# NVlabs/EmerNeRF

Measured on NVIDIA H100. Metric: training rays/sec (8192-ray batch), higher is better.
Workload: dtype f32

## Files before the change

emernerf_b200/csrc/field_fused.cu:

```cuda
#include "common.cuh"
#include "tc_common.cuh"

namespace emer {
namespace ff {

using namespace emer::tc;

constexpr int ROWS = 64;
constexpr int WGS = 3;
constexpr int THREADS = WGS * 128;
constexpr int H = 64;

struct FwdParams {
    const float* enc; int64_t ld_enc; int k_enc;
    const float *wb0, *bb0, *wb1, *bb1; int n_feat;
    const float* w0g; int64_t ld_w0;
    const float *w1h, *w1g; int64_t ld_w1;
    const float *w2, *b2;
    const float* ray_bias; int samples;
    float *sigma, *rgb;
    float *save_hb, *save_hg, *save_h1, *save_sem;
    int64_t n;
};

struct Smem {
    int wb0_hi, wb0_lo, wb1_hi, wb1_lo, wg_hi, wg_lo, w1h_hi, w1h_lo, w2_hi, w2_lo, bias, total;
};
__host__ __device__ inline Smem smem_map(int k_enc, int n_feat) {
    Smem m;
    int o = 0;
    const int wb0 = (k_enc / 4) * H * 16, wb1 = (H / 4) * n_feat * 16, wg = (H / 4) * 128 * 16, w1h = (H / 4) * H * 16,
              w2 = (H / 4) * 8 * 16;
    m.wb0_hi = o; o += wb0; m.wb0_lo = o; o += wb0;
    m.wb1_hi = o; o += wb1; m.wb1_lo = o; o += wb1;
    m.wg_hi = o; o += wg; m.wg_lo = o; o += wg;
    m.w1h_hi = o; o += w1h; m.w1h_lo = o; o += w1h;
    m.w2_hi = o; o += w2; m.w2_lo = o; o += w2;
    m.bias = o; o += (64 + 128 + 4) * 4;
    m.total = o;
    return m;
}

__device__ __forceinline__ void stage_weight(uint8_t* hi, uint8_t* lo, const float* __restrict__ w, int64_t ld, int rows,
                                             int rows_valid, int k_valid, int row0, int tid) {
    for (int e = tid; e < rows_valid * k_valid; e += THREADS) {
        const int r = e / k_valid, k = e - r * k_valid;
        float h, l;
        split(__ldg(w + (int64_t)r * ld + k), h, l);
        const int off = b_off(row0 + r, k, rows);
        *reinterpret_cast<float*>(hi + off) = h;
        *reinterpret_cast<float*>(lo + off) = l;
    }
}
__device__ __forceinline__ void stage_weight_t(uint8_t* hi, uint8_t* lo, const float* __restrict__ w, int64_t ld, int rows,
                                               int rows_valid, int k_valid, int row0, int tid) {
    for (int e = tid; e < rows_valid * k_valid; e += THREADS) {
        const int o = e / rows_valid, j = e - o * rows_valid;
        float h, l;
        split(__ldg(w + (int64_t)o * ld + j), h, l);
        const int off = b_off(row0 + j, o, rows);
        *reinterpret_cast<float*>(hi + off) = h;
        *reinterpret_cast<float*>(lo + off) = l;
    }
}

__device__ __forceinline__ float2 ld2(const float* p, bool ok) {
    return ok ? __ldg(reinterpret_cast<const float2*>(p)) : make_float2(0.f, 0.f);
}
__device__ __forceinline__ void st2(float* p, float a, float b, bool ok) {
    if (ok) *reinterpret_cast<float2*>(p) = make_float2(a, b);
}

__device__ __forceinline__ void relu_back(float (&acc)[32], const float* saved, float* dst, int64_t ld, int64_t row0,
                                          int64_t row1, bool ok0, bool ok1, int q, uint32_t (&ahi)[8][4],
                                          uint32_t (&alo)[8][4]) {
#pragma unroll
    for (int j = 0; j < 8; ++j) {
        const int c = 8 * j + 2 * q;
        const float2 m0 = ld2(saved + row0 * ld + c, ok0), m1 = ld2(saved + row1 * ld + c, ok1);
        acc[4 * j] = m0.x > 0.f ? acc[4 * j] : 0.f;
        acc[4 * j + 1] = m0.y > 0.f ? acc[4 * j + 1] : 0.f;
        acc[4 * j + 2] = m1.x > 0.f ? acc[4 * j + 2] : 0.f;
        acc[4 * j + 3] = m1.y > 0.f ? acc[4 * j + 3] : 0.f;
        st2(dst + row0 * ld + c, acc[4 * j], acc[4 * j + 1], ok0);
        st2(dst + row1 * ld + c, acc[4 * j + 2], acc[4 * j + 3], ok1);
        frag_split(acc[4 * j], acc[4 * j + 1], acc[4 * j + 2], acc[4 * j + 3], ahi[j], alo[j]);
    }
}

__device__ __forceinline__ void ray_colsum(const float (&v)[32], float* dst, int lane, bool live) {
#pragma unroll
    for (int j = 0; j < 8; ++j) {
#pragma unroll
        for (int e = 0; e < 2; ++e) {
            float s = v[4 * j + e] + v[4 * j + 2 + e];
            s += __shfl_xor_sync(0xffffffffu, s, 4);
            s += __shfl_xor_sync(0xffffffffu, s, 8);
            s += __shfl_xor_sync(0xffffffffu, s, 16);
            if (lane < 4 && live) atomicAdd(dst + 8 * j + 2 * lane + e, s);
        }
    }
}

template <int K_ENC, int NF>
__global__ void __launch_bounds__(THREADS, 1) field_fwd_kernel(const FwdParams p) {
    extern __shared__ __align__(128) uint8_t smem[];
    const Smem m = smem_map(K_ENC, NF);
    float* bias_s = reinterpret_cast<float*>(smem + m.bias);
    const int tid = threadIdx.x;

    for (int i = tid * 16; i < m.bias; i += THREADS * 16) *reinterpret_cast<float4*>(smem + i) = make_float4(0.f, 0.f, 0.f, 0.f);
    __syncthreads();
    stage_weight(smem + m.wb0_hi, smem + m.wb0_lo, p.wb0, K_ENC, H, H, K_ENC, 0, tid);
    stage_weight(smem + m.wb1_hi, smem + m.wb1_lo, p.wb1, H, NF, NF, H, 0, tid);
    stage_weight(smem + m.wg_hi, smem + m.wg_lo, p.w0g, p.ld_w0, 128, H, H, 0, tid);
    stage_weight(smem + m.wg_hi, smem + m.wg_lo, p.w1g, p.ld_w1, 128, H, H, H, tid);
    stage_weight(smem + m.w1h_hi, smem + m.w1h_lo, p.w1h, p.ld_w1, H, H, H, 0, tid);
    stage_weight(smem + m.w2_hi, smem + m.w2_lo, p.w2, H, 8, 3, H, 0, tid);
    for (int e = tid; e < 64 + 128 + 4; e += THREADS) {
        float v = 0.0f;
        if (e < 64) v = __ldg(p.bb0 + e);
        else if (e < 64 + 128) { if (e - 64 < NF) v = __ldg(p.bb1 + e - 64); }
        else if (e - 192 < 3) v = __ldg(p.b2 + e - 192);
        bias_s[e] = v;
    }
    fence_async_proxy();
    __syncthreads();

    const uint32_t sb = smem_u32(smem);
    const int wg = tid >> 7, w = (tid >> 5) & 3, lane = tid & 31, q = lane & 3;
    const float* bb0_s = bias_s;
    const float* bb1_s = bias_s + 64;
    const float* b2_s = bias_s + 192;
    const int64_t n_tiles = (p.n + ROWS - 1) / ROWS;

    for (int64_t tile = (int64_t)blockIdx.x * WGS + wg; tile < n_tiles; tile += (int64_t)gridDim.x * WGS) {
        const int64_t row0 = tile * ROWS + 16 * w + (lane >> 2), row1 = row0 + 8;
        const bool ok0 = row0 < p.n, ok1 = row1 < p.n;
        uint32_t ahi[8][4], alo[8][4];

#pragma unroll
        for (int j = 0; j < K_ENC / 8; ++j) {
            const float2 x0 = ld2(p.enc + row0 * p.ld_enc + 8 * j + 2 * q, ok0);
            const float2 x1 = ld2(p.enc + row1 * p.ld_enc + 8 * j + 2 * q, ok1);
            frag_split(x0.x, x0.y, x1.x, x1.y, ahi[j], alo[j]);
        }
        float acc[32];
        wg_fence();
#pragma unroll
        for (int ks = 0; ks < K_ENC / 8; ++ks)
            mma3<64>(acc, ahi[ks], alo[ks], b_desc(sb + m.wb0_hi, H, ks, 0), b_desc(sb + m.wb0_lo, H, ks, 0), ks > 0);
        wg_commit();
        wg_wait0();
#pragma unroll
        for (int j = 0; j < 8; ++j) {
            const int c = 8 * j + 2 * q;
            const float v0 = fmaxf(acc[4 * j] + bb0_s[c], 0.0f), v1 = fmaxf(acc[4 * j + 1] + bb0_s[c + 1], 0.0f);
            const float v2 = fmaxf(acc[4 * j + 2] + bb0_s[c], 0.0f), v3 = fmaxf(acc[4 * j + 3] + bb0_s[c + 1], 0.0f);
            if (p.save_hb) {
                st2(p.save_hb + row0 * H + c, v0, v1, ok0);
                st2(p.save_hb + row1 * H + c, v2, v3, ok1);
            }
            frag_split(v0, v1, v2, v3, ahi[j], alo[j]);
        }

        float geo[32], sem[NF > H ? 32 : 1];
        wg_fence();
#pragma unroll
        for (int ks = 0; ks < 8; ++ks) {
            mma3<64>(geo, ahi[ks], alo[ks], b_desc(sb + m.wb1_hi, NF, ks, 0), b_desc(sb + m.wb1_lo, NF, ks, 0), ks > 0);
            if constexpr (NF > H)
                mma3<64>(sem, ahi[ks], alo[ks], b_desc(sb + m.wb1_hi, NF, ks, H), b_desc(sb + m.wb1_lo, NF, ks, H), ks > 0);
        }
        wg_commit();
        wg_wait0();
#pragma unroll
        for (int j = 0; j < 8; ++j) {
            const int c = 8 * j + 2 * q;
            const float v0 = geo[4 * j] + bb1_s[c], v1 = geo[4 * j + 1] + bb1_s[c + 1];
            const float v2 = geo[4 * j + 2] + bb1_s[c], v3 = geo[4 * j + 3] + bb1_s[c + 1];
            if (j == 0 && q == 0) {
                if (ok0) p.sigma[row0] = expf(v0 - 1.0f);
                if (ok1) p.sigma[row1] = expf(v2 - 1.0f);
            }
            if (p.save_hg) {
                st2(p.save_hg + row0 * 128 + H + c, v0, v1, ok0);
                st2(p.save_hg + row1 * 128 + H + c, v2, v3, ok1);
            }
            frag_split(v0, v1, v2, v3, ahi[j], alo[j]);
        }
        if constexpr (NF > H) {
#pragma unroll
            for (int j = 0; j < 8; ++j) {
                const int c = 8 * j + 2 * q;
                st2(p.save_sem + row0 * H + c, sem[4 * j] + bb1_s[H + c], sem[4 * j + 1] + bb1_s[H + c + 1], ok0);
                st2(p.save_sem + row1 * H + c, sem[4 * j + 2] + bb1_s[H + c], sem[4 * j + 3] + bb1_s[H + c + 1], ok1);
            }
        }

        float d0[32], d1[32];
        wg_fence();
#pragma unroll
        for (int ks = 0; ks < 8; ++ks) {
            mma3<64>(d0, ahi[ks], alo[ks], b_desc(sb + m.wg_hi, 128, ks, 0), b_desc(sb + m.wg_lo, 128, ks, 0), ks > 0);
            mma3<64>(d1, ahi[ks], alo[ks], b_desc(sb + m.wg_hi, 128, ks, H), b_desc(sb + m.wg_lo, 128, ks, H), ks > 0);
        }
        wg_commit();
        wg_wait0();
        const float* rb0 = p.ray_bias + ((ok0 ? row0 : p.n - 1) / p.samples) * 128;
        const float* rb1 = p.ray_bias + ((ok1 ? row1 : p.n - 1) / p.samples) * 128;
#pragma unroll
        for (int j = 0; j < 8; ++j) {
            const int c = 8 * j + 2 * q;
            const float2 b0 = __ldg(reinterpret_cast<const float2*>(rb0 + c)), b1 = __ldg(reinterpret_cast<const float2*>(rb1 + c));
            const float v0 = fmaxf(d0[4 * j] + b0.x, 0.0f), v1 = fmaxf(d0[4 * j + 1] + b0.y, 0.0f);
            const float v2 = fmaxf(d0[4 * j + 2] + b1.x, 0.0f), v3 = fmaxf(d0[4 * j + 3] + b1.y, 0.0f);
            if (p.save_hg) {
                st2(p.save_hg + row0 * 128 + c, v0, v1, ok0);
                st2(p.save_hg + row1 * 128 + c, v2, v3, ok1);
            }
            frag_split(v0, v1, v2, v3, ahi[j], alo[j]);
        }

        wg_fence();
#pragma unroll
        for (int ks = 0; ks < 8; ++ks)
            mma3<64>(d1, ahi[ks], alo[ks], b_desc(sb + m.w1h_hi, H, ks, 0), b_desc(sb + m.w1h_lo, H, ks, 0), 1);
        wg_commit();
        wg_wait0();
#pragma unroll
        for (int j = 0; j < 8; ++j) {
            const int c = 8 * j + 2 * q;
            const float2 b0 = __ldg(reinterpret_cast<const float2*>(rb0 + H + c));
            const float2 b1 = __ldg(reinterpret_cast<const float2*>(rb1 + H + c));
            const float v0 = fmaxf(d1[4 * j] + b0.x, 0.0f), v1 = fmaxf(d1[4 * j + 1] + b0.y, 0.0f);
            const float v2 = fmaxf(d1[4 * j + 2] + b1.x, 0.0f), v3 = fmaxf(d1[4 * j + 3] + b1.y, 0.0f);
            if (p.save_h1) {
                st2(p.save_h1 + row0 * H + c, v0, v1, ok0);
                st2(p.save_h1 + row1 * H + c, v2, v3, ok1);
            }
            frag_split(v0, v1, v2, v3, ahi[j], alo[j]);
        }

        float d2[4];
        wg_fence();
#pragma unroll
        for (int ks = 0; ks < 8; ++ks)
            mma3<8>(d2, ahi[ks], alo[ks], b_desc(sb + m.w2_hi, 8, ks, 0), b_desc(sb + m.w2_lo, 8, ks, 0), ks > 0);
        wg_commit();
        wg_wait0();
#pragma unroll
        for (int e = 0; e < 2; ++e) {
            const int c = 2 * q + e;
            if (c < 3) {
                if (ok0) p.rgb[row0 * 3 + c] = 1.0f / (1.0f + expf(-(d2[e] + b2_s[c])));
                if (ok1) p.rgb[row1 * 3 + c] = 1.0f / (1.0f + expf(-(d2[2 + e] + b2_s[c])));
            }
        }
    }
}


struct BwdParams {
    const float *d_rgb, *rgb, *d_sigma, *sigma, *d_geo, *d_sem;
    const float *hb, *hg, *h1;
    const float *wb0, *wb1; int n_feat;
    const float* w0g; int64_t ld_w0; const float *w1h, *w1g; int64_t ld_w1; const float* w2;
    float *dz2, *dz1, *d1, *dzb, *d_enc; int64_t ld_denc;
    float* d_ray_bias; int samples;
    int64_t n;
};

struct BSmem {
    int w2_hi, w2_lo, w1_hi, w1_lo, w0_hi, w0_lo, wb1_hi, wb1_lo, wb0_hi, wb0_lo, total;
};
__host__ __device__ inline BSmem bsmem_map(int k_enc, int n_feat) {
    BSmem m;
    int o = 0;
    const int w2 = (8 / 4) * H * 16, w1 = (H / 4) * 128 * 16, w0 = (H / 4) * H * 16, wb1 = (n_feat / 4) * H * 16,
              wb0 = (H / 4) * k_enc * 16;
    m.w2_hi = o; o += w2; m.w2_lo = o; o += w2;
    m.w1_hi = o; o += w1; m.w1_lo = o; o += w1;
    m.w0_hi = o; o += w0; m.w0_lo = o; o += w0;
    m.wb1_hi = o; o += wb1; m.wb1_lo = o; o += wb1;
    m.wb0_hi = o; o += wb0; m.wb0_lo = o; o += wb0;
    m.total = o;
    return m;
}

template <int K_ENC, int NF>
__global__ void __launch_bounds__(THREADS, 1) field_bwd_kernel(const BwdParams p) {
    extern __shared__ __align__(128) uint8_t smem[];
    const BSmem m = bsmem_map(K_ENC, NF);
    const int tid = threadIdx.x;
    for (int i = tid * 16; i < m.total; i += THREADS * 16) *reinterpret_cast<float4*>(smem + i) = make_float4(0.f, 0.f, 0.f, 0.f);
    __syncthreads();
    stage_weight_t(smem + m.w2_hi, smem + m.w2_lo, p.w2, H, H, H, 3, 0, tid);
    stage_weight_t(smem + m.w1_hi, smem + m.w1_lo, p.w1h, p.ld_w1, 128, H, H, 0, tid);
    stage_weight_t(smem + m.w1_hi, smem + m.w1_lo, p.w1g, p.ld_w1, 128, H, H, H, tid);
    stage_weight_t(smem + m.w0_hi, smem + m.w0_lo, p.w0g, p.ld_w0, H, H, H, 0, tid);
    stage_weight_t(smem + m.wb1_hi, smem + m.wb1_lo, p.wb1, H, H, H, NF, 0, tid);
    stage_weight_t(smem + m.wb0_hi, smem + m.wb0_lo, p.wb0, K_ENC, K_ENC, K_ENC, H, 0, tid);
    fence_async_proxy();
    __syncthreads();

    const uint32_t sb = smem_u32(smem);
    const int wg = tid >> 7, w = (tid >> 5) & 3, lane = tid & 31, q = lane & 3;
    const bool ray_sums = p.d_ray_bias != nullptr && (p.samples % 32 == 0);
    const int64_t n_tiles = (p.n + ROWS - 1) / ROWS;

    for (int64_t tile = (int64_t)blockIdx.x * WGS + wg; tile < n_tiles; tile += (int64_t)gridDim.x * WGS) {
        const int64_t wrow0 = tile * ROWS + 16 * w;
        const int64_t row0 = wrow0 + (lane >> 2), row1 = row0 + 8;
        const bool ok0 = row0 < p.n, ok1 = row1 < p.n;
        const bool warp_live = wrow0 < p.n;
        float* rbias = ray_sums ? p.d_ray_bias + (wrow0 / p.samples) * 128 : nullptr;
        uint32_t ahi[8][4], alo[8][4];

        {
            float v[4] = {0.f, 0.f, 0.f, 0.f};
#pragma unroll
            for (int e = 0; e < 4; ++e) {
                const int c = 2 * q + (e & 1);
                const int64_t row = (e < 2) ? row0 : row1;
                if (c < 3 && (e < 2 ? ok0 : ok1) && p.d_rgb) {
                    const float y = __ldg(p.rgb + row * 3 + c);
                    v[e] = __ldg(p.d_rgb + row * 3 + c) * (y * (1.0f - y));
                    if (p.dz2) p.dz2[row * 3 + c] = v[e];
                }
            }
            frag_split(v[0], v[1], v[2], v[3], ahi[0], alo[0]);
        }
        float acc[32];
        wg_fence();
        mma3<64>(acc, ahi[0], alo[0], b_desc(sb + m.w2_hi, H, 0, 0), b_desc(sb + m.w2_lo, H, 0, 0), 0);
        wg_commit();
        wg_wait0();

        relu_back(acc, p.h1, p.dz1, H, row0, row1, ok0, ok1, q, ahi, alo);
        if (ray_sums) ray_colsum(acc, rbias + H, lane, warp_live);

        float dg[32];
        wg_fence();
#pragma unroll
        for (int ks = 0; ks < 8; ++ks) {
            mma3<64>(acc, ahi[ks], alo[ks], b_desc(sb + m.w1_hi, 128, ks, 0), b_desc(sb + m.w1_lo, 128, ks, 0), ks > 0);
            mma3<64>(dg, ahi[ks], alo[ks], b_desc(sb + m.w1_hi, 128, ks, H), b_desc(sb + m.w1_lo, 128, ks, H), ks > 0);
        }
        wg_commit();
        wg_wait0();
        relu_back(acc, p.hg, p.d1, 128, row0, row1, ok0, ok1, q, ahi, alo);
        if (ray_sums) ray_colsum(acc, rbias, lane, warp_live);

        wg_fence();
#pragma unroll
        for (int ks = 0; ks < 8; ++ks)
            mma3<64>(dg, ahi[ks], alo[ks], b_desc(sb + m.w0_hi, H, ks, 0), b_desc(sb + m.w0_lo, H, ks, 0), 1);
        wg_commit();
        wg_wait0();
#pragma unroll
        for (int j = 0; j < 8; ++j) {
            const int c = 8 * j + 2 * q;
            float v0 = dg[4 * j], v1 = dg[4 * j + 1], v2 = dg[4 * j + 2], v3 = dg[4 * j + 3];
            if (p.d_geo) {
                const float2 g0 = ld2(p.d_geo + row0 * H + c, ok0), g1 = ld2(p.d_geo + row1 * H + c, ok1);
                v0 += g0.x; v1 += g0.y; v2 += g1.x; v3 += g1.y;
            }
            if (j == 0 && q == 0 && p.d_sigma) {
                if (ok0) v0 += __ldg(p.d_sigma + row0) * fminf(__ldg(p.sigma + row0), 3269017.25f);
                if (ok1) v2 += __ldg(p.d_sigma + row1) * fminf(__ldg(p.sigma + row1), 3269017.25f);
            }
            st2(p.d1 + row0 * 128 + H + c, v0, v1, ok0);
            st2(p.d1 + row1 * 128 + H + c, v2, v3, ok1);
            frag_split(v0, v1, v2, v3, ahi[j], alo[j]);
        }

        wg_fence();
#pragma unroll
        for (int ks = 0; ks < 8; ++ks)
            mma3<64>(acc, ahi[ks], alo[ks], b_desc(sb + m.wb1_hi, H, ks, 0), b_desc(sb + m.wb1_lo, H, ks, 0), ks > 0);
        wg_commit();
        wg_wait0();
        if constexpr (NF > H) {
            if (p.d_sem) {
#pragma unroll
                for (int j = 0; j < 8; ++j) {
                    const int c = 8 * j + 2 * q;
                    const float2 s0 = ld2(p.d_sem + row0 * H + c, ok0), s1 = ld2(p.d_sem + row1 * H + c, ok1);
                    frag_split(s0.x, s0.y, s1.x, s1.y, ahi[j], alo[j]);
                }
                wg_fence();
#pragma unroll
                for (int ks = 0; ks < 8; ++ks)
                    mma3<64>(acc, ahi[ks], alo[ks], b_desc(sb + m.wb1_hi, H, 8 + ks, 0), b_desc(sb + m.wb1_lo, H, 8 + ks, 0), 1);
                wg_commit();
                wg_wait0();
            }
        }
        relu_back(acc, p.hb, p.dzb, H, row0, row1, ok0, ok1, q, ahi, alo);

        if (p.d_enc) {
            float de[K_ENC / 2];
            wg_fence();
#pragma unroll
            for (int ks = 0; ks < 8; ++ks)
                mma3<K_ENC>(de, ahi[ks], alo[ks], b_desc(sb + m.wb0_hi, K_ENC, ks, 0), b_desc(sb + m.wb0_lo, K_ENC, ks, 0), ks > 0);
            wg_commit();
            wg_wait0();
#pragma unroll
            for (int j = 0; j < K_ENC / 8; ++j) {
                const int c = 8 * j + 2 * q;
                st2(p.d_enc + row0 * p.ld_denc + c, de[4 * j], de[4 * j + 1], ok0);
                st2(p.d_enc + row1 * p.ld_denc + c, de[4 * j + 2], de[4 * j + 3], ok1);
            }
        }
    }
}

}
}

using namespace emer;

extern "C" int emer_field_fwd(const float* enc, int64_t ld_enc, int k_enc, const float* wb0, const float* bb0,
                              const float* wb1, const float* bb1, int n_feat, const float* w0g, int64_t ld_w0,
                              const float* w1h, const float* w1g, int64_t ld_w1, const float* w2, const float* b2,
                              const float* ray_bias, int samples, float* sigma, float* rgb, float* save_hb, float* save_hg,
                              float* save_h1, float* save_sem, int64_t n, void* stream) {
    using namespace emer::ff;
    if (n == 0) return 0;
    EMER_REQUIRE(enc && wb0 && bb0 && wb1 && bb1 && w0g && w1h && w1g && w2 && b2 && ray_bias && sigma && rgb,
                 "emer_field_fwd: NULL pointer");
    EMER_REQUIRE(k_enc == 32 || k_enc == 40 || k_enc == 64, "emer_field_fwd: k_enc=%d (L*F of the grid) must be 32, 40 or 64", k_enc);
    EMER_REQUIRE(n_feat == 64 || n_feat == 128, "emer_field_fwd: n_feat=%d must be 64 or 128", n_feat);
    EMER_REQUIRE(samples > 0, "emer_field_fwd: samples per ray must be positive");
    EMER_REQUIRE(ld_enc % 8 == 0 && ((uintptr_t)enc & 31) == 0, "emer_field_fwd: enc rows must be 32-byte aligned");
    EMER_REQUIRE(((uintptr_t)ray_bias & 15) == 0, "emer_field_fwd: ray_bias must be 16-byte aligned");
    EMER_REQUIRE((((uintptr_t)save_hb | (uintptr_t)save_hg | (uintptr_t)save_h1 | (uintptr_t)save_sem) & 31) == 0,
                 "emer_field_fwd: save buffers must be 32-byte aligned");
    EMER_REQUIRE(n_feat == 64 || save_sem, "emer_field_fwd: the semantic half needs its output buffer");
    FwdParams p{};
    p.enc = enc; p.ld_enc = ld_enc; p.k_enc = k_enc; p.wb0 = wb0; p.bb0 = bb0; p.wb1 = wb1; p.bb1 = bb1; p.n_feat = n_feat;
    p.w0g = w0g; p.ld_w0 = ld_w0; p.w1h = w1h; p.w1g = w1g; p.ld_w1 = ld_w1; p.w2 = w2; p.b2 = b2;
    p.ray_bias = ray_bias; p.samples = samples; p.sigma = sigma; p.rgb = rgb;
    p.save_hb = save_hb; p.save_hg = save_hg; p.save_h1 = save_h1; p.save_sem = save_sem; p.n = n;
    const Smem m = smem_map(k_enc, n_feat);
    size_t smem = (size_t)m.total;
    EMER_REQUIRE(smem <= 227 * 1024, "emer_field_fwd: %zu B of shared memory needed", smem);
    const int64_t n_tiles = ceil_div(n, ROWS);
    int64_t grid = sm_count();
    if (grid > ceil_div(n_tiles, WGS)) grid = ceil_div(n_tiles, WGS);
    auto launch = [&](auto kernel, size_t& configured) -> int {
        if (smem > configured) {
            cudaError_t e = cudaFuncSetAttribute(kernel, cudaFuncAttributeMaxDynamicSharedMemorySize, (int)smem);
            if (e != cudaSuccess) {
                set_error("emer_field_fwd: cudaFuncSetAttribute(%zu): %s", smem, cudaGetErrorString(e));
                return -2;
            }
            configured = smem;
        }
        kernel<<<(unsigned)grid, THREADS, smem, (cudaStream_t)stream>>>(p);
        return 0;
    };
    static size_t configured_dev[6][64] = {{0}};
    const int dev = current_device();
    int rc;
    if (n_feat == 64) {
        if (k_enc == 32) rc = launch(field_fwd_kernel<32, 64>, configured_dev[0][dev]);
        else if (k_enc == 40) rc = launch(field_fwd_kernel<40, 64>, configured_dev[1][dev]);
        else rc = launch(field_fwd_kernel<64, 64>, configured_dev[2][dev]);
    } else {
        if (k_enc == 32) rc = launch(field_fwd_kernel<32, 128>, configured_dev[3][dev]);
        else if (k_enc == 40) rc = launch(field_fwd_kernel<40, 128>, configured_dev[4][dev]);
        else rc = launch(field_fwd_kernel<64, 128>, configured_dev[5][dev]);
    }
    if (rc) return rc;
    return check_launch("emer_field_fwd");
}

extern "C" int emer_field_bwd(const float* d_rgb, const float* rgb, const float* d_sigma, const float* sigma,
                              const float* d_geo, const float* d_sem, const float* hb, const float* hg, const float* h1,
                              const float* wb0, int k_enc, const float* wb1, int n_feat, const float* w0g, int64_t ld_w0,
                              const float* w1h, const float* w1g, int64_t ld_w1, const float* w2, float* dz2, float* dz1,
                              float* d1, float* dzb, float* d_enc, int64_t ld_denc, float* d_ray_bias, int samples,
                              int64_t n, void* stream) {
    using namespace emer::ff;
    if (n == 0) return 0;
    EMER_REQUIRE(rgb && sigma && hb && hg && h1 && wb0 && wb1 && w0g && w1h && w1g && w2 && dz1 && d1 && dzb,
                 "emer_field_bwd: NULL pointer");
    EMER_REQUIRE(k_enc == 32 || k_enc == 40 || k_enc == 64, "emer_field_bwd: k_enc=%d must be 32, 40 or 64", k_enc);
    EMER_REQUIRE(n_feat == 64 || n_feat == 128, "emer_field_bwd: n_feat=%d must be 64 or 128", n_feat);
    EMER_REQUIRE(samples > 0, "emer_field_bwd: samples per ray must be positive");
    EMER_REQUIRE(!d_enc || (ld_denc % 8 == 0 && ld_denc >= k_enc), "emer_field_bwd: d_enc rows must be 32-byte aligned");
    EMER_REQUIRE((((uintptr_t)hb | (uintptr_t)hg | (uintptr_t)h1 | (uintptr_t)dz1 | (uintptr_t)d1 | (uintptr_t)dzb |
                   (uintptr_t)d_enc | (uintptr_t)d_geo | (uintptr_t)d_sem) & 31) == 0,
                 "emer_field_bwd: row buffers must be 32-byte aligned");
    EMER_REQUIRE(!d_ray_bias || samples % 32 == 0, "emer_field_bwd: per-ray sums need samples %% 32 == 0 (got %d)", samples);
    BwdParams p{};
    p.d_rgb = d_rgb; p.rgb = rgb; p.d_sigma = d_sigma; p.sigma = sigma; p.d_geo = d_geo; p.d_sem = d_sem;
    p.hb = hb; p.hg = hg; p.h1 = h1; p.wb0 = wb0; p.wb1 = wb1; p.n_feat = n_feat;
    p.w0g = w0g; p.ld_w0 = ld_w0; p.w1h = w1h; p.w1g = w1g; p.ld_w1 = ld_w1; p.w2 = w2;
    p.dz2 = dz2; p.dz1 = dz1; p.d1 = d1; p.dzb = dzb; p.d_enc = d_enc; p.ld_denc = ld_denc; p.d_ray_bias = d_ray_bias; p.samples = samples;
    p.n = n;
    const BSmem m = bsmem_map(k_enc, n_feat);
    size_t smem = (size_t)m.total;
    EMER_REQUIRE(smem <= 227 * 1024, "emer_field_bwd: %zu B of shared memory needed", smem);
    const int64_t n_tiles = ceil_div(n, ROWS);
    int64_t grid = sm_count();
    if (grid > ceil_div(n_tiles, WGS)) grid = ceil_div(n_tiles, WGS);
    auto launch = [&](auto kernel, size_t& configured) -> int {
        if (smem > configured) {
            cudaError_t e = cudaFuncSetAttribute(kernel, cudaFuncAttributeMaxDynamicSharedMemorySize, (int)smem);
            if (e != cudaSuccess) {
                set_error("emer_field_bwd: cudaFuncSetAttribute(%zu): %s", smem, cudaGetErrorString(e));
                return -2;
            }
            configured = smem;
        }
        kernel<<<(unsigned)grid, THREADS, smem, (cudaStream_t)stream>>>(p);
        return 0;
    };
    static size_t configured_dev[6][64] = {{0}};
    const int dev = current_device();
    int rc;
    if (n_feat == 64) {
        if (k_enc == 32) rc = launch(field_bwd_kernel<32, 64>, configured_dev[0][dev]);
        else if (k_enc == 40) rc = launch(field_bwd_kernel<40, 64>, configured_dev[1][dev]);
        else rc = launch(field_bwd_kernel<64, 64>, configured_dev[2][dev]);
    } else {
        if (k_enc == 32) rc = launch(field_bwd_kernel<32, 128>, configured_dev[3][dev]);
        else if (k_enc == 40) rc = launch(field_bwd_kernel<40, 128>, configured_dev[4][dev]);
        else rc = launch(field_bwd_kernel<64, 128>, configured_dev[5][dev]);
    }
    if (rc) return rc;
    return check_launch("emer_field_bwd");
}
```

emernerf_b200/csrc/field_wgrad.cu:

```cuda
#include "common.cuh"
#include "tc_common.cuh"

namespace emer {
namespace fw {

using namespace emer::tc;

constexpr int TR = 16;
constexpr int STAGES = 4;
constexpr int THREADS = 384;
constexpr int MIN_TILES = 4;

constexpr int PANEL64 = TR * 64 * 4, PANEL8 = TR * 8 * 4;
constexpr int P_DZB = 0, P_DF = 2 * PANEL64, P_DSEM = 4 * PANEL64, P_DZ0 = 6 * PANEL64, P_DZ1 = 8 * PANEL64,
              P_DZ2 = 10 * PANEL64, P_BYTES = P_DZ2 + 2 * PANEL8;

template <int KE, bool HEAD>
struct Stage {
    static constexpr int LD_ENC = KE + 4, LD64 = 68, LD128 = 132, LD_D1 = HEAD ? LD128 : LD64;
    static constexpr int ENC = 0, HB = ENC + TR * LD_ENC, DZB = HB + TR * LD64, DSEM = DZB + TR * LD64,
                         D1 = DSEM + TR * LD64, DF = D1 + (HEAD ? 64 : 0), HG = D1 + TR * LD_D1, H1 = HG + TR * LD128,
                         DZ1 = H1 + TR * LD64, DZ2 = DZ1 + TR * LD64;
    static constexpr int FLOATS = HEAD ? DZ2 + TR * 3 : HG;
};

struct Params {
    const float* enc; int64_t ld_enc;
    const float *hb, *hg, *h1, *dz2, *dz1, *d1, *dzb, *d_sem;
    float *dwb0, *dbb0, *dwb1, *dbb1;
    float *dw0g, *dw1h, *dw1g; int64_t ld_w0, ld_w1;
    float *dw2, *db2;
    int64_t n;
};

__device__ __forceinline__ void cp_async16(float* dst, const float* src, int bytes) {
    asm volatile("cp.async.cg.shared.global [%0], [%1], 16, %2;\n" ::"r"(smem_u32(dst)), "l"(src), "r"(bytes) : "memory");
}
__device__ __forceinline__ void cp_async_commit() { asm volatile("cp.async.commit_group;\n" ::: "memory"); }
template <int N>
__device__ __forceinline__ void cp_async_wait() { asm volatile("cp.async.wait_group %0;\n" ::"n"(N) : "memory"); }

template <int W>
__device__ __forceinline__ void copy_rows(float* dst, const float* src, int64_t ld, int64_t row0, int64_t n) {
    constexpr int CPR = W / 4;
    for (int c = threadIdx.x; c < TR * CPR; c += THREADS) {
        const int r = c / CPR, j = c % CPR;
        const bool ok = row0 + r < n;
        cp_async16(dst + r * (W + 4) + 4 * j, ok ? src + (row0 + r) * ld + 4 * j : src, ok ? 16 : 0);
    }
}

template <int FV>
__device__ __forceinline__ void load_a(const float* x, int ld, int f0, int q, uint32_t (&hi)[2][4], uint32_t (&lo)[2][4]) {
    const int f1 = f0 + 8;
#pragma unroll
    for (int ks = 0; ks < 2; ++ks) {
        const float* ra = x + (8 * ks + 2 * q) * ld;
        const float* rb = ra + ld;
        frag_split(f0 < FV ? ra[f0] : 0.0f, f0 < FV ? rb[f0] : 0.0f, f1 < FV ? ra[f1] : 0.0f, f1 < FV ? rb[f1] : 0.0f,
                   hi[ks], lo[ks]);
    }
}

template <int N>
__device__ __forceinline__ void mma_tile(float (&acc)[N / 2], const uint32_t (&hi)[2][4], const uint32_t (&lo)[2][4],
                                         uint32_t panel) {
#pragma unroll
    for (int ks = 0; ks < 2; ++ks)
        mma3<N>(acc, hi[ks], lo[ks], b_desc(panel, N, ks, 0), b_desc(panel + TR * N * 4, N, ks, 0), 1);
}

template <int N>
__device__ __forceinline__ void flush(const float (&acc)[N / 2], float* dw, int64_t ld, int fv, int ov, int f0, int q) {
#pragma unroll
    for (int j = 0; j < N / 8; ++j) {
#pragma unroll
        for (int e = 0; e < 4; ++e) {
            const int f = e < 2 ? f0 : f0 + 8, o = 8 * j + 2 * q + (e & 1);
            if (f < fv && o < ov) atomicAdd(dw + (int64_t)o * ld + f, acc[4 * j + e]);
        }
    }
}

template <int KE, bool HEAD>
__global__ void __launch_bounds__(THREADS, 1) field_wgrad_kernel(const __grid_constant__ Params p) {
    using S = Stage<KE, HEAD>;
    extern __shared__ __align__(128) uint8_t smem[];
    float* ring = reinterpret_cast<float*>(smem + P_BYTES);
    const uint32_t pan = smem_u32(smem);
    const int tid = threadIdx.x, lane = tid & 31, q = lane & 3;
    const int wgi = __shfl_sync(0xffffffffu, tid >> 7, 0);
    const int f0 = 16 * ((tid >> 5) & 3) + (lane >> 2);
    const bool sem = p.d_sem != nullptr;
    const int64_t n_tiles = (p.n + TR - 1) / TR;
    const int64_t my_tiles = (n_tiles - blockIdx.x + gridDim.x - 1) / gridDim.x;

    auto issue = [&](int64_t i) {
        if (i < my_tiles) {
            const int64_t row0 = (blockIdx.x + i * gridDim.x) * TR;
            float* st = ring + (i % STAGES) * S::FLOATS;
            copy_rows<KE>(st + S::ENC, p.enc, p.ld_enc, row0, p.n);
            copy_rows<64>(st + S::HB, p.hb, 64, row0, p.n);
            copy_rows<64>(st + S::DZB, p.dzb, 64, row0, p.n);
            if (sem) copy_rows<64>(st + S::DSEM, p.d_sem, 64, row0, p.n);
            copy_rows<HEAD ? 128 : 64>(st + S::D1, p.d1 + (HEAD ? 0 : 64), 128, row0, p.n);
            if constexpr (HEAD) {
                copy_rows<128>(st + S::HG, p.hg, 128, row0, p.n);
                copy_rows<64>(st + S::H1, p.h1, 64, row0, p.n);
                copy_rows<64>(st + S::DZ1, p.dz1, 64, row0, p.n);
                if (tid < TR * 3 / 4) {
                    const int64_t left = (p.n - row0 < TR ? p.n - row0 : TR) * 12 - 16 * tid;
                    const int b = left <= 0 ? 0 : (left < 16 ? (int)left : 16);
                    cp_async16(st + S::DZ2 + 4 * tid, b ? p.dz2 + row0 * 3 + 4 * tid : p.dz2, b);
                }
            }
        }
        cp_async_commit();
    };

    const int col = tid & 63;
    int soff = -1, sld = S::LD64, rows = 64;
    uint32_t pb = 0;
    float* db = nullptr;
    bool real = true;
    switch (tid >> 6) {
        case 0: soff = S::DZB; pb = P_DZB; db = p.dbb0; break;
        case 1: soff = S::DF; sld = S::LD_D1; pb = P_DF; db = p.dbb1; break;
        case 2: if (sem) { soff = S::DSEM; pb = P_DSEM; db = p.dbb1 + 64; } break;
        case 3: if (HEAD) { soff = S::D1; sld = S::LD_D1; pb = P_DZ0; } break;
        case 4: if (HEAD) { soff = S::DZ1; pb = P_DZ1; } break;
        default:
            if (HEAD && col < 8) { soff = S::DZ2; sld = 3; rows = 8; pb = P_DZ2; db = p.db2; real = col < 3; }
            break;
    }

    float a0[32], a1[32], a2[4], dbs = 0.0f;
#pragma unroll
    for (int i = 0; i < 32; ++i) a0[i] = a1[i] = 0.0f;
#pragma unroll
    for (int i = 0; i < 4; ++i) a2[i] = 0.0f;

#pragma unroll
    for (int s = 0; s < STAGES - 1; ++s) issue(s);
    for (int64_t i = 0; i < my_tiles; ++i) {
        cp_async_wait<STAGES - 2>();
        __syncthreads();
        issue(i + STAGES - 1);
        const float* st = ring + (i % STAGES) * S::FLOATS;
        if (soff >= 0) {
            const float* z = st + soff + (real ? col : 0);
#pragma unroll
            for (int ks = 0; ks < 2; ++ks) {
#pragma unroll
                for (int h = 0; h < 2; ++h) {
                    float v[4], hi[4], lo[4];
#pragma unroll
                    for (int j = 0; j < 4; ++j) {
                        v[j] = real ? z[(8 * ks + 2 * j + h) * sld] : 0.0f;
                        split(v[j], hi[j], lo[j]);
                        dbs += v[j];
                    }
                    uint8_t* dst = smem + pb + (2 * ks + h) * rows * 16 + col * 16;
                    *reinterpret_cast<float4*>(dst) = make_float4(hi[0], hi[1], hi[2], hi[3]);
                    *reinterpret_cast<float4*>(dst + TR * rows * 4) = make_float4(lo[0], lo[1], lo[2], lo[3]);
                }
            }
        }
        fence_async_proxy();
        __syncthreads();

        uint32_t h0[2][4], l0[2][4], h1[2][4], l1[2][4];
        if (wgi == 0) {
            load_a<KE>(st + S::ENC, S::LD_ENC, f0, q, h0, l0);
            load_a<64>(st + S::HB, S::LD64, f0, q, h1, l1);
            wg_fence();
            mma_tile<64>(a0, h0, l0, pan + P_DZB);
            mma_tile<64>(a1, h1, l1, pan + P_DF);
            wg_commit();
            wg_wait0();
        } else if (wgi == 1) {
            if constexpr (HEAD) {
                load_a<64>(st + S::HG + 64, S::LD128, f0, q, h0, l0);
                load_a<64>(st + S::H1, S::LD64, f0, q, h1, l1);
                wg_fence();
                mma_tile<64>(a0, h0, l0, pan + P_DZ0);
                mma_tile<64>(a1, h0, l0, pan + P_DZ1);
                mma_tile<8>(a2, h1, l1, pan + P_DZ2);
                wg_commit();
                wg_wait0();
            }
        } else if (HEAD || sem) {
            if (HEAD) load_a<64>(st + S::HG, S::LD128, f0, q, h0, l0);
            if (sem) load_a<64>(st + S::HB, S::LD64, f0, q, h1, l1);
            wg_fence();
            if (HEAD) mma_tile<64>(a0, h0, l0, pan + P_DZ1);
            if (sem) mma_tile<64>(a1, h1, l1, pan + P_DSEM);
            wg_commit();
            wg_wait0();
        }
    }
    cp_async_wait<0>();

    if (wgi == 0) {
        flush<64>(a0, p.dwb0, KE, KE, 64, f0, q);
        flush<64>(a1, p.dwb1, 64, 64, 64, f0, q);
    } else if (wgi == 1) {
        if (HEAD) {
            flush<64>(a0, p.dw0g, p.ld_w0, 64, 64, f0, q);
            flush<64>(a1, p.dw1g, p.ld_w1, 64, 64, f0, q);
            flush<8>(a2, p.dw2, 64, 64, 3, f0, q);
        }
    } else {
        if (HEAD) flush<64>(a0, p.dw1h, p.ld_w1, 64, 64, f0, q);
        if (sem) flush<64>(a1, p.dwb1 + 64 * 64, 64, 64, 64, f0, q);
    }
    if (db && real) atomicAdd(db + col, dbs);
}

template <int KE, bool HEAD>
static int launch_t(const Params& p, cudaStream_t st) {
    constexpr int smem = P_BYTES + STAGES * Stage<KE, HEAD>::FLOATS * 4;
    static_assert(smem <= 227 * 1024, "field_wgrad_kernel: shared memory");
    static bool configured[64] = {false};
    const int dev = current_device();
    if (!configured[dev]) {
        cudaError_t e = cudaFuncSetAttribute(field_wgrad_kernel<KE, HEAD>, cudaFuncAttributeMaxDynamicSharedMemorySize, smem);
        if (e != cudaSuccess) {
            set_error("emer_field_wgrad: cudaFuncSetAttribute(%d): %s", smem, cudaGetErrorString(e));
            return -2;
        }
        configured[dev] = true;
    }
    int64_t grid = sm_count();
    const int64_t ctas = ceil_div(ceil_div(p.n, TR), MIN_TILES);
    if (grid > ctas) grid = ctas;
    field_wgrad_kernel<KE, HEAD><<<(unsigned)grid, THREADS, smem, st>>>(p);
    return check_launch("emer_field_wgrad");
}

template <bool HEAD>
static int launch_h(const Params& p, int k_enc, cudaStream_t st) {
    if (k_enc == 32) return launch_t<32, HEAD>(p, st);
    if (k_enc == 40) return launch_t<40, HEAD>(p, st);
    return launch_t<64, HEAD>(p, st);
}

}
}

extern "C" int emer_field_wgrad(const float* enc, int64_t ld_enc, int k_enc, const float* hb, const float* hg,
                                const float* h1, const float* dz2, const float* dz1, const float* d1, const float* dzb,
                                const float* d_sem, int n_feat, float* dwb0, float* dbb0, float* dwb1, float* dbb1,
                                float* dw0g, int64_t ld_w0, float* dw1h, float* dw1g, int64_t ld_w1, float* dw2,
                                float* db2, int64_t n, void* stream) {
    if (n == 0) return 0;
    EMER_REQUIRE(enc && hb && d1 && dzb && dwb0 && dbb0 && dwb1 && dbb1, "emer_field_wgrad: NULL pointer");
    EMER_REQUIRE(!dz2 || (hg && h1 && dz1 && dw0g && dw1h && dw1g && dw2 && db2),
                 "emer_field_wgrad: NULL pointer among the colour head's buffers");
    EMER_REQUIRE(k_enc == 32 || k_enc == 40 || k_enc == 64, "emer_field_wgrad: k_enc=%d must be 32, 40 or 64", k_enc);
    EMER_REQUIRE(n_feat == 64 || n_feat == 128, "emer_field_wgrad: n_feat=%d must be 64 or 128", n_feat);
    EMER_REQUIRE(!d_sem || n_feat == 128, "emer_field_wgrad: d_sem needs n_feat = 128");
    EMER_REQUIRE(ld_enc % 4 == 0 && ld_enc >= k_enc, "emer_field_wgrad: ld_enc=%lld (need a multiple of 4, >= k_enc)",
                 (long long)ld_enc);
    EMER_REQUIRE(!dz2 || (ld_w0 >= 64 && ld_w1 >= 64), "emer_field_wgrad: ld_w0=%lld ld_w1=%lld shorter than a block",
                 (long long)ld_w0, (long long)ld_w1);
    EMER_REQUIRE((((uintptr_t)enc | (uintptr_t)hb | (uintptr_t)hg | (uintptr_t)h1 | (uintptr_t)dz2 | (uintptr_t)dz1 |
                   (uintptr_t)d1 | (uintptr_t)dzb | (uintptr_t)d_sem) & 15) == 0,
                 "emer_field_wgrad: row buffers must be 16-byte aligned");
    emer::fw::Params p{enc, ld_enc, hb, hg, h1, dz2, dz1, d1, dzb, d_sem, dwb0, dbb0, dwb1, dbb1,
                       dw0g, dw1h, dw1g, ld_w0, ld_w1, dw2, db2, n};
    const cudaStream_t st = (cudaStream_t)stream;
    return dz2 ? emer::fw::launch_h<true>(p, k_enc, st) : emer::fw::launch_h<false>(p, k_enc, st);
}
```

Baseline: 2.296 million.

## Warp-specialize field weight-grad kernel into producer/consumer with double-buffered panels

The weight-gradient kernel is restructured so one warpgroup becomes a producer: it issues cp.async loads, splits gradient columns into hi/lo panels and accumulates bias sums. The other two warpgroups consume those panels with wgmma. Named barriers and a double-buffered panel area replace the block-wide __syncthreads, and setmaxnreg moves registers from the producer to the consumers. The ring drops to three stages to make room for the second panel buffer. The forward field kernel also uses clamped unconditional loads for the encoding and issues the semantic-head MMA as its own group before the geometry MMA, which lowers accumulator register pressure. This adds barrier-protocol complexity and risks deadlock or races if the arrive/sync counts are wrong.

After: 2.380 million (median of 6 runs). 3.7% higher.

```diff
diff --git a/emernerf_b200/csrc/field_fused.cu b/emernerf_b200/csrc/field_fused.cu
--- a/emernerf_b200/csrc/field_fused.cu
+++ b/emernerf_b200/csrc/field_fused.cu
@@ -139,10 +139,12 @@
         const bool ok0 = row0 < p.n, ok1 = row1 < p.n;
         uint32_t ahi[8][4], alo[8][4];
 
+        const float* x0p = p.enc + (ok0 ? row0 : p.n - 1) * p.ld_enc + 2 * q;
+        const float* x1p = p.enc + (ok1 ? row1 : p.n - 1) * p.ld_enc + 2 * q;
 #pragma unroll
         for (int j = 0; j < K_ENC / 8; ++j) {
-            const float2 x0 = ld2(p.enc + row0 * p.ld_enc + 8 * j + 2 * q, ok0);
-            const float2 x1 = ld2(p.enc + row1 * p.ld_enc + 8 * j + 2 * q, ok1);
+            const float2 x0 = __ldg(reinterpret_cast<const float2*>(x0p + 8 * j));
+            const float2 x1 = __ldg(reinterpret_cast<const float2*>(x1p + 8 * j));
             frag_split(x0.x, x0.y, x1.x, x1.y, ahi[j], alo[j]);
         }
         float acc[32];
@@ -164,14 +166,26 @@
             frag_split(v0, v1, v2, v3, ahi[j], alo[j]);
         }
 
-        float geo[32], sem[NF > H ? 32 : 1];
-        wg_fence();
-#pragma unroll
-        for (int ks = 0; ks < 8; ++ks) {
+        if constexpr (NF > H) {
+            float sem[32];
+            wg_fence();
+#pragma unroll
+            for (int ks = 0; ks < 8; ++ks)
+                mma3<64>(sem, ahi[ks], alo[ks], b_desc(sb + m.wb1_hi, NF, ks, H), b_desc(sb + m.wb1_lo, NF, ks, H), ks > 0);
+            wg_commit();
+            wg_wait0();
+#pragma unroll
+            for (int j = 0; j < 8; ++j) {
+                const int c = 8 * j + 2 * q;
+                st2(p.save_sem + row0 * H + c, sem[4 * j] + bb1_s[H + c], sem[4 * j + 1] + bb1_s[H + c + 1], ok0);
+                st2(p.save_sem + row1 * H + c, sem[4 * j + 2] + bb1_s[H + c], sem[4 * j + 3] + bb1_s[H + c + 1], ok1);
+            }
+        }
+        float geo[32];
+        wg_fence();
+#pragma unroll
+        for (int ks = 0; ks < 8; ++ks)
             mma3<64>(geo, ahi[ks], alo[ks], b_desc(sb + m.wb1_hi, NF, ks, 0), b_desc(sb + m.wb1_lo, NF, ks, 0), ks > 0);
-            if constexpr (NF > H)
-                mma3<64>(sem, ahi[ks], alo[ks], b_desc(sb + m.wb1_hi, NF, ks, H), b_desc(sb + m.wb1_lo, NF, ks, H), ks > 0);
-        }
         wg_commit();
         wg_wait0();
 #pragma unroll
@@ -188,14 +202,6 @@
                 st2(p.save_hg + row1 * 128 + H + c, v2, v3, ok1);
             }
             frag_split(v0, v1, v2, v3, ahi[j], alo[j]);
-        }
-        if constexpr (NF > H) {
-#pragma unroll
-            for (int j = 0; j < 8; ++j) {
-                const int c = 8 * j + 2 * q;
-                st2(p.save_sem + row0 * H + c, sem[4 * j] + bb1_s[H + c], sem[4 * j + 1] + bb1_s[H + c + 1], ok0);
-                st2(p.save_sem + row1 * H + c, sem[4 * j + 2] + bb1_s[H + c], sem[4 * j + 3] + bb1_s[H + c + 1], ok1);
-            }
         }
 
         float d0[32], d1[32];
diff --git a/emernerf_b200/csrc/field_wgrad.cu b/emernerf_b200/csrc/field_wgrad.cu
--- a/emernerf_b200/csrc/field_wgrad.cu
+++ b/emernerf_b200/csrc/field_wgrad.cu
@@ -7,9 +7,12 @@
 using namespace emer::tc;
 
 constexpr int TR = 16;
-constexpr int STAGES = 4;
+constexpr int STAGES = 3;
 constexpr int THREADS = 384;
+constexpr int PROD_REGS = 56, CONS_REGS = 224;
 constexpr int MIN_TILES = 4;
+
+constexpr int BAR_FULL = 1, BAR_EMPTY = 3, BAR_RING = 5, BAR_PROD = 5 + STAGES;
 
 constexpr int PANEL64 = TR * 64 * 4, PANEL8 = TR * 8 * 4;
 constexpr int P_DZB = 0, P_DF = 2 * PANEL64, P_DSEM = 4 * PANEL64, P_DZ0 = 6 * PANEL64, P_DZ1 = 8 * PANEL64,
@@ -39,14 +42,50 @@
 __device__ __forceinline__ void cp_async_commit() { asm volatile("cp.async.commit_group;\n" ::: "memory"); }
 template <int N>
 __device__ __forceinline__ void cp_async_wait() { asm volatile("cp.async.wait_group %0;\n" ::"n"(N) : "memory"); }
+__device__ __forceinline__ void bar_sync(int id, int count) { asm volatile("bar.sync %0, %1;\n" ::"r"(id), "r"(count) : "memory"); }
+__device__ __forceinline__ void bar_arrive(int id, int count) { asm volatile("bar.arrive %0, %1;\n" ::"r"(id), "r"(count) : "memory"); }
 
 template <int W>
-__device__ __forceinline__ void copy_rows(float* dst, const float* src, int64_t ld, int64_t row0, int64_t n) {
-    constexpr int CPR = W / 4;
-    for (int c = threadIdx.x; c < TR * CPR; c += THREADS) {
-        const int r = c / CPR, j = c % CPR;
-        const bool ok = row0 + r < n;
-        cp_async16(dst + r * (W + 4) + 4 * j, ok ? src + (row0 + r) * ld + 4 * j : src, ok ? 16 : 0);
+__device__ __forceinline__ void copy_rows(float* dst, const float* src, int64_t ld, int64_t row0, int rows_left, int t) {
+    constexpr int CPR = W / 4, CHUNKS = TR * CPR;
+    const float* s = src + row0 * ld;
+#pragma unroll
+    for (int k = 0; k < (CHUNKS + 127) / 128; ++k) {
+        const int c = t + 128 * k;
+        if (CHUNKS % 128 == 0 || c < CHUNKS) {
+            const int r = c / CPR, j = c % CPR;
+            const bool ok = r < rows_left;
+            cp_async16(dst + r * (W + 4) + 4 * j, ok ? s + r * ld + 4 * j : src, ok ? 16 : 0);
+        }
+    }
+}
+
+template <int B, int KE, bool HEAD>
+__device__ __forceinline__ void split_col(const float* st, uint8_t* pan, int col, bool sem, float& dbs) {
+    using S = Stage<KE, HEAD>;
+    constexpr int soff = B == 0 ? S::DZB : B == 1 ? S::DF : B == 2 ? S::DSEM : B == 3 ? S::D1 : B == 4 ? S::DZ1 : S::DZ2;
+    constexpr int sld = B == 1 || B == 3 ? S::LD_D1 : (B == 5 ? 3 : S::LD64);
+    constexpr int rows = B == 5 ? 8 : 64;
+    constexpr int pb = B == 0 ? P_DZB : B == 1 ? P_DF : B == 2 ? P_DSEM : B == 3 ? P_DZ0 : B == 4 ? P_DZ1 : P_DZ2;
+    if constexpr (B >= 3 && !HEAD) return;
+    if ((B == 2 && !sem) || (B == 5 && col >= 8)) return;
+    const bool real = B != 5 || col < 3;
+    const float* z = st + soff + (real ? col : 0);
+#pragma unroll
+    for (int ks = 0; ks < 2; ++ks) {
+#pragma unroll
+        for (int h = 0; h < 2; ++h) {
+            float v[4], hi[4], lo[4];
+#pragma unroll
+            for (int j = 0; j < 4; ++j) {
+                v[j] = real ? z[(8 * ks + 2 * j + h) * sld] : 0.0f;
+                split(v[j], hi[j], lo[j]);
+                dbs += v[j];
+            }
+            uint8_t* dst = pan + pb + (2 * ks + h) * rows * 16 + col * 16;
+            *reinterpret_cast<float4*>(dst) = make_float4(hi[0], hi[1], hi[2], hi[3]);
+            *reinterpret_cast<float4*>(dst + TR * rows * 4) = make_float4(lo[0], lo[1], lo[2], lo[3]);
+        }
     }
 }
 
@@ -86,140 +125,140 @@
 __global__ void __launch_bounds__(THREADS, 1) field_wgrad_kernel(const __grid_constant__ Params p) {
     using S = Stage<KE, HEAD>;
     extern __shared__ __align__(128) uint8_t smem[];
-    float* ring = reinterpret_cast<float*>(smem + P_BYTES);
-    const uint32_t pan = smem_u32(smem);
+    float* ring = reinterpret_cast<float*>(smem + 2 * P_BYTES);
     const int tid = threadIdx.x, lane = tid & 31, q = lane & 3;
     const int wgi = __shfl_sync(0xffffffffu, tid >> 7, 0);
-    const int f0 = 16 * ((tid >> 5) & 3) + (lane >> 2);
     const bool sem = p.d_sem != nullptr;
     const int64_t n_tiles = (p.n + TR - 1) / TR;
     const int64_t my_tiles = (n_tiles - blockIdx.x + gridDim.x - 1) / gridDim.x;
 
-    auto issue = [&](int64_t i) {
-        if (i < my_tiles) {
-            const int64_t row0 = (blockIdx.x + i * gridDim.x) * TR;
-            float* st = ring + (i % STAGES) * S::FLOATS;
-            copy_rows<KE>(st + S::ENC, p.enc, p.ld_enc, row0, p.n);
-            copy_rows<64>(st + S::HB, p.hb, 64, row0, p.n);
-            copy_rows<64>(st + S::DZB, p.dzb, 64, row0, p.n);
-            if (sem) copy_rows<64>(st + S::DSEM, p.d_sem, 64, row0, p.n);
-            copy_rows<HEAD ? 128 : 64>(st + S::D1, p.d1 + (HEAD ? 0 : 64), 128, row0, p.n);
-            if constexpr (HEAD) {
-                copy_rows<128>(st + S::HG, p.hg, 128, row0, p.n);
-                copy_rows<64>(st + S::H1, p.h1, 64, row0, p.n);
-                copy_rows<64>(st + S::DZ1, p.dz1, 64, row0, p.n);
-                if (tid < TR * 3 / 4) {
-                    const int64_t left = (p.n - row0 < TR ? p.n - row0 : TR) * 12 - 16 * tid;
-                    const int b = left <= 0 ? 0 : (left < 16 ? (int)left : 16);
-                    cp_async16(st + S::DZ2 + 4 * tid, b ? p.dz2 + row0 * 3 + 4 * tid : p.dz2, b);
+    if (wgi == 0) {
+        asm volatile("setmaxnreg.dec.sync.aligned.u32 %0;\n" ::"n"(PROD_REGS));
+        auto issue = [&](int64_t i, int slot) {
+            if (i < my_tiles) {
+                const int64_t row0 = (blockIdx.x + i * gridDim.x) * TR;
+                const int rows_left = p.n - row0 < TR ? (int)(p.n - row0) : TR;
+                float* st = ring + slot * S::FLOATS;
+                copy_rows<KE>(st + S::ENC, p.enc, p.ld_enc, row0, rows_left, tid);
+                copy_rows<64>(st + S::HB, p.hb, 64, row0, rows_left, tid);
+                copy_rows<64>(st + S::DZB, p.dzb, 64, row0, rows_left, tid);
+                if (sem) copy_rows<64>(st + S::DSEM, p.d_sem, 64, row0, rows_left, tid);
+                copy_rows<HEAD ? 128 : 64>(st + S::D1, p.d1 + (HEAD ? 0 : 64), 128, row0, rows_left, tid);
+                if constexpr (HEAD) {
+                    copy_rows<128>(st + S::HG, p.hg, 128, row0, rows_left, tid);
+                    copy_rows<64>(st + S::H1, p.h1, 64, row0, rows_left, tid);
+                    copy_rows<64>(st + S::DZ1, p.dz1, 64, row0, rows_left, tid);
+                    if (tid < TR * 3 / 4) {
+                        const int left = rows_left * 12 - 16 * tid;
+                        const int b = left <= 0 ? 0 : (left < 16 ? left : 16);
+                        cp_async16(st + S::DZ2 + 4 * tid, b ? p.dz2 + row0 * 3 + 4 * tid : p.dz2, b);
+                    }
                 }
             }
-        }
-        cp_async_commit();
-    };
-
-    const int col = tid & 63;
-    int soff = -1, sld = S::LD64, rows = 64;
-    uint32_t pb = 0;
-    float* db = nullptr;
-    bool real = true;
-    switch (tid >> 6) {
-        case 0: soff = S::DZB; pb = P_DZB; db = p.dbb0; break;
-        case 1: soff = S::DF; sld = S::LD_D1; pb = P_DF; db = p.dbb1; break;
-        case 2: if (sem) { soff = S::DSEM; pb = P_DSEM; db = p.dbb1 + 64; } break;
-        case 3: if (HEAD) { soff = S::D1; sld = S::LD_D1; pb = P_DZ0; } break;
-        case 4: if (HEAD) { soff = S::DZ1; pb = P_DZ1; } break;
-        default:
-            if (HEAD && col < 8) { soff = S::DZ2; sld = 3; rows = 8; pb = P_DZ2; db = p.db2; real = col < 3; }
-            break;
-    }
-
-    float a0[32], a1[32], a2[4], dbs = 0.0f;
-#pragma unroll
-    for (int i = 0; i < 32; ++i) a0[i] = a1[i] = 0.0f;
-#pragma unroll
-    for (int i = 0; i < 4; ++i) a2[i] = 0.0f;
-
-#pragma unroll
-    for (int s = 0; s < STAGES - 1; ++s) issue(s);
-    for (int64_t i = 0; i < my_tiles; ++i) {
-        cp_async_wait<STAGES - 2>();
-        __syncthreads();
-        issue(i + STAGES - 1);
-        const float* st = ring + (i % STAGES) * S::FLOATS;
-        if (soff >= 0) {
-            const float* z = st + soff + (real ? col : 0);
-#pragma unroll
-            for (int ks = 0; ks < 2; ++ks) {
-#pragma unroll
-                for (int h = 0; h < 2; ++h) {
-                    float v[4], hi[4], lo[4];
-#pragma unroll
-                    for (int j = 0; j < 4; ++j) {
-                        v[j] = real ? z[(8 * ks + 2 * j + h) * sld] : 0.0f;
-                        split(v[j], hi[j], lo[j]);
-                        dbs += v[j];
-                    }
-                    uint8_t* dst = smem + pb + (2 * ks + h) * rows * 16 + col * 16;
-                    *reinterpret_cast<float4*>(dst) = make_float4(hi[0], hi[1], hi[2], hi[3]);
-                    *reinterpret_cast<float4*>(dst + TR * rows * 4) = make_float4(lo[0], lo[1], lo[2], lo[3]);
+            cp_async_commit();
+        };
+        const int col = tid & 63, half = __shfl_sync(0xffffffffu, tid >> 6, 0);
+        float db0 = 0.0f, db1 = 0.0f, db2 = 0.0f;
+        issue(0, 0);
+        issue(1, 1);
+        int slot = 0;
+        for (int64_t i = 0; i < my_tiles; ++i, slot = slot + 1 == STAGES ? 0 : slot + 1) {
+            const int pb = (int)(i & 1), prev = slot == 0 ? STAGES - 1 : slot - 1;
+            if (i >= 1 && i + 2 < my_tiles) bar_sync(BAR_RING + prev, THREADS);
+            issue(i + 2, prev);
+            if (i >= 2) bar_sync(BAR_EMPTY + pb, THREADS);
+            cp_async_wait<2>();
+            bar_sync(BAR_PROD, 128);
+            const float* st = ring + slot * S::FLOATS;
+            uint8_t* pan = smem + pb * P_BYTES;
+            if (half == 0) {
+                split_col<0, KE, HEAD>(st, pan, col, sem, db0);
+                split_col<2, KE, HEAD>(st, pan, col, sem, db1);
+                split_col<4, KE, HEAD>(st, pan, col, sem, db2);
+            } else {
+                split_col<1, KE, HEAD>(st, pan, col, sem, db0);
+                split_col<3, KE, HEAD>(st, pan, col, sem, db1);
+                split_col<5, KE, HEAD>(st, pan, col, sem, db2);
+            }
+            fence_async_proxy();
+            bar_arrive(BAR_FULL + pb, THREADS);
+        }
+        cp_async_wait<0>();
+        if (half == 0) {
+            atomicAdd(p.dbb0 + col, db0);
+            if (sem) atomicAdd(p.dbb1 + 64 + col, db1);
+        } else {
+            atomicAdd(p.dbb1 + col, db0);
+            if (HEAD && col < 3) atomicAdd(p.db2 + col, db2);
+        }
+    } else {
+        asm volatile("setmaxnreg.inc.sync.aligned.u32 %0;\n" ::"n"(CONS_REGS));
+        const uint32_t pan0 = smem_u32(smem);
+        const int f0 = 16 * ((tid >> 5) & 3) + (lane >> 2);
+        float a0[32], a1[32], a2[32], a3[4];
+#pragma unroll
+        for (int i = 0; i < 32; ++i) a0[i] = a1[i] = a2[i] = 0.0f;
+#pragma unroll
+        for (int i = 0; i < 4; ++i) a3[i] = 0.0f;
+
+        int slot = 0;
+        for (int64_t i = 0; i < my_tiles; ++i, slot = slot + 1 == STAGES ? 0 : slot + 1) {
+            const int pb = (int)(i & 1);
+            bar_sync(BAR_FULL + pb, THREADS);
+            const float* st = ring + slot * S::FLOATS;
+            const uint32_t pan = pan0 + (uint32_t)pb * P_BYTES;
+            uint32_t h0[2][4], l0[2][4], h1[2][4], l1[2][4], h2[2][4], l2[2][4];
+            if (wgi == 1) {
+                load_a<KE>(st + S::ENC, S::LD_ENC, f0, q, h0, l0);
+                if (HEAD) load_a<64>(st + S::HG + 64, S::LD128, f0, q, h1, l1);
+            } else {
+                load_a<64>(st + S::HB, S::LD64, f0, q, h0, l0);
+                if (HEAD) {
+                    load_a<64>(st + S::HG, S::LD128, f0, q, h1, l1);
+                    load_a<64>(st + S::H1, S::LD64, f0, q, h2, l2);
                 }
             }
-        }
-        fence_async_proxy();
-        __syncthreads();
-
-        uint32_t h0[2][4], l0[2][4], h1[2][4], l1[2][4];
-        if (wgi == 0) {
-            load_a<KE>(st + S::ENC, S::LD_ENC, f0, q, h0, l0);
-            load_a<64>(st + S::HB, S::LD64, f0, q, h1, l1);
+            if (i + STAGES < my_tiles) bar_arrive(BAR_RING + slot, THREADS);
             wg_fence();
-            mma_tile<64>(a0, h0, l0, pan + P_DZB);
-            mma_tile<64>(a1, h1, l1, pan + P_DF);
+            if (wgi == 1) {
+                mma_tile<64>(a0, h0, l0, pan + P_DZB);
+                if (HEAD) {
+                    mma_tile<64>(a1, h1, l1, pan + P_DZ0);
+                    mma_tile<64>(a2, h1, l1, pan + P_DZ1);
+                }
+            } else {
+                mma_tile<64>(a0, h0, l0, pan + P_DF);
+                if (sem) mma_tile<64>(a2, h0, l0, pan + P_DSEM);
+                if (HEAD) {
+                    mma_tile<64>(a1, h1, l1, pan + P_DZ1);
+                    mma_tile<8>(a3, h2, l2, pan + P_DZ2);
+                }
+            }
             wg_commit();
             wg_wait0();
-        } else if (wgi == 1) {
-            if constexpr (HEAD) {
-                load_a<64>(st + S::HG + 64, S::LD128, f0, q, h0, l0);
-                load_a<64>(st + S::H1, S::LD64, f0, q, h1, l1);
-                wg_fence();
-                mma_tile<64>(a0, h0, l0, pan + P_DZ0);
-                mma_tile<64>(a1, h0, l0, pan + P_DZ1);
-                mma_tile<8>(a2, h1, l1, pan + P_DZ2);
-                wg_commit();
-                wg_wait0();
-            }
-        } else if (HEAD || sem) {
-            if (HEAD) load_a<64>(st + S::HG, S::LD128, f0, q, h0, l0);
-            if (sem) load_a<64>(st + S::HB, S::LD64, f0, q, h1, l1);
-            wg_fence();
-            if (HEAD) mma_tile<64>(a0, h0, l0, pan + P_DZ1);
-            if (sem) mma_tile<64>(a1, h1, l1, pan + P_DSEM);
-            wg_commit();
-            wg_wait0();
-        }
-    }
-    cp_async_wait<0>();
-
-    if (wgi == 0) {
-        flush<64>(a0, p.dwb0, KE, KE, 64, f0, q);
-        flush<64>(a1, p.dwb1, 64, 64, 64, f0, q);
-    } else if (wgi == 1) {
-        if (HEAD) {
-            flush<64>(a0, p.dw0g, p.ld_w0, 64, 64, f0, q);
-            flush<64>(a1, p.dw1g, p.ld_w1, 64, 64, f0, q);
-            flush<8>(a2, p.dw2, 64, 64, 3, f0, q);
-        }
-    } else {
-        if (HEAD) flush<64>(a0, p.dw1h, p.ld_w1, 64, 64, f0, q);
-        if (sem) flush<64>(a1, p.dwb1 + 64 * 64, 64, 64, 64, f0, q);
-    }
-    if (db && real) atomicAdd(db + col, dbs);
+            if (i + 2 < my_tiles) bar_arrive(BAR_EMPTY + pb, THREADS);
+        }
+
+        if (wgi == 1) {
+            flush<64>(a0, p.dwb0, KE, KE, 64, f0, q);
+            if (HEAD) {
+                flush<64>(a1, p.dw0g, p.ld_w0, 64, 64, f0, q);
+                flush<64>(a2, p.dw1g, p.ld_w1, 64, 64, f0, q);
+            }
+        } else {
+            flush<64>(a0, p.dwb1, 64, 64, 64, f0, q);
+            if (sem) flush<64>(a2, p.dwb1 + 64 * 64, 64, 64, 64, f0, q);
+            if (HEAD) {
+                flush<64>(a1, p.dw1h, p.ld_w1, 64, 64, f0, q);
+                flush<8>(a3, p.dw2, 64, 64, 3, f0, q);
+            }
+        }
+    }
 }
 
 template <int KE, bool HEAD>
 static int launch_t(const Params& p, cudaStream_t st) {
-    constexpr int smem = P_BYTES + STAGES * Stage<KE, HEAD>::FLOATS * 4;
+    constexpr int smem = 2 * P_BYTES + STAGES * Stage<KE, HEAD>::FLOATS * 4;
     static_assert(smem <= 227 * 1024, "field_wgrad_kernel: shared memory");
     static bool configured[64] = {false};
     const int dev = current_device();
```
